# syl051088/DynaAlign

Hardware: AMD Instinct MI355X
Metric: sequence-pairs/sec (MinHash k=4 n_hash=500; NW BLOSUM62) at 1/2/4/8 MI355X (higher is better)
Workload: dtype u32

## Files before the change

### dynaalign_amd/csrc/api.cpp

```cpp
#include <sched.h>

#include <algorithm>
#include <atomic>
#include <chrono>
#include <climits>
#include <cmath>
#include <condition_variable>
#include <cstddef>
#include <map>
#include <memory>
#include <cstdlib>
#include <cstring>
#include <functional>
#include <mutex>
#include <random>
#include <string>
#include <thread>
#include <vector>

#include "da_common.hpp"

namespace da { size_t destroy_cached_comms(); }

namespace da {
// ... 306 lines not shown

double now_ms() { return std::chrono::duration<double, std::milli>(std::chrono::steady_clock::now().time_since_epoch()).count(); }

size_t block_budget() {
  size_t free_b = 0, total_b = 0;
  if (hipMemGetInfo(&free_b, &total_b) != hipSuccess) free_b = (size_t)8 << 30;
  {
    int dev = 0;
    (void)hipGetDevice(&dev);
    std::lock_guard<std::mutex> g(big_cache().m);
    for (const auto &e : big_cache().parked) if (e.dev == dev) free_b += e.bytes;
  }
  size_t budget = free_b / 2;
  if (da::config().block_bytes) budget = (size_t)da::config().block_bytes;
  return budget;
}
int64_t block_rows(int64_t n, size_t bytes_per_elem) {
  int64_t rows = (int64_t)(block_budget() / ((size_t)n * bytes_per_elem));
  rows = rows / 128 * 128;
  if (rows < 128) rows = 128;
  return rows;
}
int64_t rows_per_block(int64_t n, size_t bytes_per_elem) { return std::min(block_rows(n, bytes_per_elem), n); }

}
}

using namespace da;

namespace da {
namespace {
bool env_flag(const char *name) { return getenv(name) != nullptr; }
int64_t env_i64(const char *name, int64_t dflt) { const char *e = getenv(name); return e ? atoll(e) : dflt; }
uint64_t env_u64(const char *name, uint64_t dflt) { const char *e = getenv(name); return e ? strtoull(e, nullptr, 10) : dflt; }
enum MhExpand { MH_EXPAND_DEFAULT, MH_EXPAND_ROWS, MH_EXPAND_ROWSPIPE, MH_EXPAND_PIPE, MH_EXPAND_TILES };
Config parse_config() {
  Config c;
  c.mh_no_dedup = env_flag("DYNAALIGN_MH_NO_DEDUP");
  c.mh_no_sparse = env_flag("DYNAALIGN_MH_NO_SPARSE");
  c.mh_no_pipe = env_flag("DYNAALIGN_MH_NO_PIPE");
  c.mh_pipe_one_stream = env_flag("DYNAALIGN_MH_PIPE_ONE_STREAM");
  c.mh_dedup_min_n = env_i64("DYNAALIGN_MH_DEDUP_MIN_N", -1);
  c.mh_dedup_max_pct = env_i64("DYNAALIGN_MH_DEDUP_MAX_PCT", -1);
  c.mh_sparse_max_pairs = std::min<uint64_t>(env_u64("DYNAALIGN_MH_SPARSE_MAX_PAIRS", 400000000ull), 0xfffffff0ull);
  c.mh_no_hybrid = env_flag("DYNAALIGN_MH_NO_HYBRID");
  c.mh_hybrid_min_n = env_i64("DYNAALIGN_MH_HYBRID_MIN_N", -1);
  c.mh_hybrid_dedup = env_flag("DYNAALIGN_MH_HYBRID_DEDUP");
  if (const char *e = getenv("DYNAALIGN_MH_EXPAND"))
    c.mh_expand = !strcmp(e, "rows") ? MH_EXPAND_ROWS : !strcmp(e, "rowspipe") ? MH_EXPAND_ROWSPIPE : !strcmp(e, "pipe") ? MH_EXPAND_PIPE
                : !strcmp(e, "tiles") ? MH_EXPAND_TILES : MH_EXPAND_DEFAULT;
  c.mh_pipe_step = (int)std::max<int64_t>(0, env_i64("DYNAALIGN_MH_PIPE_STEP", 0));
  c.mh_pipe_wg = (int)std::max<int64_t>(0, std::min<int64_t>(4, env_i64("DYNAALIGN_MH_PIPE_WG", 0)));
  c.mh_pipe_head = (int)std::max<int64_t>(0, env_i64("DYNAALIGN_MH_PIPE_HEAD", 0));
  const int pb = (int)env_i64("DYNAALIGN_PLANE_BITS", 0);
  c.plane_bits = (pb == 32 || pb == 16 || pb == 15 || pb == 14 || pb == 12) ? pb : 0;
  c.k2_no_asm = env_flag("DYNAALIGN_K2_NO_ASM");
  c.k2_persist = env_flag("DYNAALIGN_K2_PERSIST");
  c.k2_wg_per_cu = (int)std::max<int64_t>(0, env_i64("DYNAALIGN_K2_WG_PER_CU", 0));
  c.nw_no_dedup = env_flag("DYNAALIGN_NW_NO_DEDUP");
  c.nw_int32 = env_flag("DYNAALIGN_NW_INT32");
  c.nw_no_prefix = env_flag("DYNAALIGN_NW_NO_PREFIX_SHARE");
  c.nw_dedup_min_n = env_i64("DYNAALIGN_NW_DEDUP_MIN_N", -1);
  c.no_host_widen = env_flag("DYNAALIGN_NO_HOST_WIDEN");
  c.plain_d2h = env_flag("DYNAALIGN_PLAIN_D2H");
  c.no_buffer_cache = env_flag("DYNAALIGN_NO_BUFFER_CACHE");
  c.d2h_threads = (int)std::max<int64_t>(0, env_i64("DYNAALIGN_D2H_THREADS", 0));
  c.buffer_cache_pct = (int)std::max<int64_t>(0, std::min<int64_t>(90, env_i64("DYNAALIGN_BUFFER_CACHE_PCT", 30)));
  c.block_bytes = env_u64("DYNAALIGN_BLOCK_BYTES", 0);
  c.trace = env_flag("DYNAALIGN_TRACE");
  c.louvain_debug = env_flag("DYNAALIGN_LOUVAIN_DEBUG");
  c.louvain_threads = (int)std::max<int64_t>(0, env_i64("DYNAALIGN_LOUVAIN_THREADS", 0));
  return c;
}
std::atomic<const Config *> g_config{nullptr};
}
const Config &config() {
  const Config *c = g_config.load(std::memory_order_acquire);
  if (!c) {
    const Config *fresh = new Config(parse_config());
    if (g_config.compare_exchange_strong(c, fresh, std::memory_order_acq_rel)) c = fresh;
    else delete fresh;
  }
  return *c;
}
}
extern "C" void da_config_reload(void) { da::g_config.store(new da::Config(da::parse_config()), std::memory_order_release); }

extern "C" {

const char *da_last_error(void) { return last_error_ref().c_str(); }

const char *da_status_message(int status) {
  switch (status) {
    case DA_ERR_EMPTY_INPUT: return "Input sequences vector cannot be empty";
    case DA_ERR_BAD_K: return "'k' must be a positive integer";
    case DA_ERR_BAD_NHASH: return "Number of hash functions must be positive";
    case DA_ERR_BAD_MATRIX: return "Invalid substitution matrix name: %s";
    case DA_ERR_BAD_RESIDUE_SEQ1: return "Invalid amino acid in sequence1: %c";
    case DA_ERR_BAD_RESIDUE_SEQ2: return "Invalid amino acid in sequence2: %c";
    case DA_ERR_NOMEM: return "out of memory";
    case DA_ERR_NO_DEVICE: return "no usable HIP device";
    case DA_ERR_HIP: return "HIP runtime error";
    case DA_ERR_UNSUPPORTED: return "unsupported by the gfx950 kernels";
    case DA_ERR_BAD_ARG: return "bad argument";
    default: return "";
  }
// ... 244 lines not shown
  const uint16_t *dense = nullptr, *rare = nullptr;
  unsigned long long st[4] = {0, 0, 0, 0};
  if ((rc = split_ok ? launch_mh_heavy_split(d_work, n, n_hash, dict.max_ids, HY_KEEP, &dense, &rare, d_stats, stream)
                     : launch_mh_sparse_count(ids, ld_ids, n, n_hash, dict.max_ids, d_stats, stream)) != DA_OK) return rc;
  DA_HIP_TRY(hipMemcpyAsync(split_ok ? st : st + 2, d_stats, split_ok ? sizeof(st) : 16, hipMemcpyDeviceToHost, stream));
  DA_HIP_TRY(hipStreamSynchronize(stream));
  const double pairs_all = 0.5 * (double)n * (double)(n - 1);
  if (sparse_ok && st[2] <= mh_sparse_pairs_limit() && st[3] <= 4096 && (double)st[2] <= pairs_all * (double)n_hash / 5000.0)
    *a = MhAdmission{MhOperand::sparse, st[2], ids, nullptr, ld_ids};
  else if (split_ok && st[0] <= mh_sparse_pairs_limit() && st[1] <= 4096 && (double)st[0] <= pairs_all * (double)n_hash / 25000.0)
    *a = MhAdmission{MhOperand::split, st[0], rare, dense, ld_ids};
  return DA_OK;
}
struct MhCodes {
  DevBuf sig, planes, pwork, scratch, entries32, entries;
  int64_t m = 0;
  int n_hash = 0, bits = 32;
  Dictionary dict;
  MhAdmission adm;
  bool split() const { return adm.form == MhOperand::split; }
  int lists(hipStream_t st) const {
    return launch_mh_sparse_lists(adm.codes, adm.ld_ids, m, n_hash, dict.max_ids, adm.pairs, scratch.as<uint32_t>(), entries32.as<uint32_t>(), entries.as<uint16_t>(), st);
  }
  int fixup(int kind, void *out, int64_t ld_out, hipStream_t st, int64_t tr0 = 0, int64_t tr1 = -1) const {
    return launch_mh_sparse_fixup(scratch.as<uint32_t>(), entries.as<uint16_t>(), m, n_hash, dict.max_ids, adm.ld_ids, kind, out, ld_out, tr0,
                                  tr1 < 0 ? (m + 127) / 128 : tr1, st);
  }
};
static int mh_codes(const uint8_t *d_res, const int64_t *d_off, int64_t m, int k, int n_hash, const uint32_t *d_seeds, bool ask_sparse,
                    int split_from_bits, MhCodes *c, hipStream_t stream) {
  int rc;
  const int64_t lds = sig_ld_for(n_hash);
  const size_t wb = mh_planes_workspace_bytes(m, n_hash);
  c->m = m; c->n_hash = n_hash;
  if ((rc = c->sig.alloc((size_t)m * lds * sizeof(uint32_t))) != DA_OK || (rc = c->planes.alloc((size_t)mh_planes_words(m, n_hash) * sizeof(uint32_t))) != DA_OK ||
      (rc = c->pwork.alloc(wb)) != DA_OK) return rc;
  uint32_t *sig = c->sig.as<uint32_t>(), *planes = c->planes.as<uint32_t>();
  if ((rc = launch_minhash_signatures(d_res, d_off, m, k, n_hash, d_seeds, sig, lds, stream)) != DA_OK) return rc;
  const int min_bits = env_plane_bits();
  const Dictionary &dict = c->dict;
  if ((rc = run_dictionary(sig, lds, m, n_hash, min_bits, c->pwork.p, wb, &c->dict, stream)) != DA_OK) return rc;
  if ((rc = mh_admit(dict, c->pwork.p, m, n_hash, ask_sparse, split_from_bits, &c->adm, stream)) != DA_OK) return rc;
  if (c->adm.form != MhOperand::dense &&
      (c->scratch.alloc(mh_sparse_scratch_words(m, n_hash, dict.max_ids, c->adm.ld_ids) * 4) != DA_OK ||
       c->entries32.alloc((size_t)c->adm.pairs * 4 + 16) != DA_OK || c->entries.alloc((size_t)c->adm.pairs * 2 + 16) != DA_OK)) {
    (void)hipGetLastError();
    c->scratch.release(); c->entries32.release(); c->entries.release();
    c->adm = MhAdmission();
  }
  if (c->adm.form == MhOperand::sparse) { c->bits = 0; return DA_OK; }
  if (c->split()) { c->bits = 8; return launch_ids_to_planes(c->pwork.p, m, n_hash, 8, planes, stream, c->adm.dense); }
  return planes_from(dict, sig, lds, m, n_hash, min_bits, c->pwork.p, planes, &c->bits, stream);
}
struct MhCall {
  int64_t n; int n_hash; double *out; int64_t ld; hipStream_t stream; MhRoute &route; const MhEvents &ev; const MhCodes &c; const MhDedup &d;
  uint16_t *dtab = nullptr; int64_t ld_d = 0; void *ex = nullptr; bool pk = false;
};
constexpr int MH_NO_PIPE = -1;
static int mh_finish(const MhCall &k, int last_event, MhForm taken, int steps) {
  DA_HIP_TRY(hipEventRecord(k.ev[last_event], k.stream));
  DA_HIP_TRY(hipStreamSynchronize(k.stream));
  k.route.taken = taken; k.ev.steps(k.route, steps);
  return DA_OK;
}
static int mh_sparse(const MhCall &k) {
  const MhCodes &c = k.c;
  int rc;
  if ((rc = launch_mh_sparse(c.adm.codes, c.adm.ld_ids, k.n, k.n_hash, c.dict.max_ids, c.adm.pairs, c.scratch.as<uint32_t>(), c.entries32.as<uint32_t>(),
                             c.entries.as<uint16_t>(), k.out, k.ld, k.stream, k.ev[3])) != DA_OK || (rc = mh_finish(k, 4, MH_SPARSE, 3)) != DA_OK) return rc;
  k.route.unique = (int64_t)c.adm.pairs;
  MhEvents::ms(k.route, 4, k.ev[3], k.ev[4]);
  return DA_OK;
}
static int mh_direct(const MhCall &k) {
  const MhCodes &c = k.c;
  int rc;
  const PipeLease lease(1, c.split());
  PipeRes *const pr = lease.r;
  if (pr) {
    DA_HIP_TRY(hipStreamWaitEvent(pr->side, k.ev[2], 0));
    if ((rc = c.lists(pr->side)) != DA_OK) return rc;
    DA_HIP_TRY(hipEventRecord(pr->ev[0], pr->side));
  } else if (c.split() && (rc = c.lists(k.stream)) != DA_OK) return rc;
  if ((rc = launch_mh_compare(c.planes.as<uint32_t>(), k.n, k.n_hash, 0, k.n, true, DA_OUT_F64, k.out, k.ld, k.stream, c.bits)) != DA_OK) return rc;
  if (pr) DA_HIP_TRY(hipStreamWaitEvent(k.stream, pr->ev[0], 0));
  if (c.split() && (rc = c.fixup(DA_OUT_F64, k.out, k.ld, k.stream)) != DA_OK) return rc;
  return mh_finish(k, 3, MH_DIRECT, 3);
}
static int mh_one_stream(const MhCall &k) {
  const MhCodes &c = k.c;
  int rc;
  if (c.split() && (rc = c.lists(k.stream)) != DA_OK) return rc;
  if ((rc = k.pk ? launch_mh_compare_pk(c.planes.as<uint32_t>(), k.d.U, k.n_hash, reinterpret_cast<uint8_t *>(k.dtab), k.stream)
                 : launch_mh_compare(c.planes.as<uint32_t>(), k.d.U, k.n_hash, 0, k.d.U, true, DA_OUT_COMPACT, k.dtab, k.ld_d, k.stream, c.bits)) != DA_OK)
    return rc;
  if (c.split() && (rc = c.fixup(DA_OUT_COMPACT, k.dtab, k.ld_d, k.stream)) != DA_OK) return rc;
  DA_HIP_TRY(hipEventRecord(k.ev[3], k.stream));
  if ((rc = k.d.rows ? launch_expand_stream(k.dtab, k.ld_d, k.d.p.uidx, k.n, k.d.U, k.n_hash, k.out, k.ld, k.ex, k.stream, k.ev[4], k.pk)
                     : launch_expand_unique(k.dtab, k.ld_d, k.d.p.uidx, k.n, DA_OUT_F64, false, k.n_hash, k.out, k.ld, k.stream, 0,
                                            static_cast<uint16_t *>(k.ex), k.d.p.ufirst, k.d.U, k.ev[4], k.ev[5])) != DA_OK) return rc;
  k.route.chunks = k.route.expand_launches = 1;
  return k.d.rows ? mh_finish(k, 5, MH_ROWS, 5) : mh_finish(k, 6, MH_TILES, 6);
}
static int mh_rows_pipe(const MhCall &k) {
  const Config &cfg = da::config();
  const MhCodes &c = k.c;
  const int64_t U = k.d.U, KB = mh_sym_bands(U);
  const hipStream_t stream = k.stream;
  int rc;
  const bool two = expand_stream_packed(k.n_hash);
  const int wg = cfg.mh_pipe_wg > 0 ? cfg.mh_pipe_wg : two ? 2 : 1, head = cfg.mh_pipe_head > 0 ? cfg.mh_pipe_head : two ? 1 : 4,
            step = cfg.mh_pipe_step > 0 ? cfg.mh_pipe_step : two ? 8 : 4;
  const bool alt = !cfg.mh_pipe_one_stream;
  std::vector<int64_t> cuts{0};
  while (cuts.back() < KB) cuts.push_back(std::min(KB, cuts.back() + (cuts.size() == 1 ? head : step)));
  const size_t C = cuts.size() - 1;
  const PipeLease lease(3 * C + 2);
  PipeRes *const pr = lease.r;
  if (!pr) return MH_NO_PIPE;
  hipEvent_t *pe = pr->ev.data();
  DA_HIP_TRY(hipStreamWaitEvent(pr->side, k.ev[2], 0));
  if ((rc = launch_mh_compare_edges_u16(c.planes.as<uint32_t>(), U, k.n_hash, k.dtab, k.ld_d, stream, c.bits, k.pk)) != DA_OK) return rc;
  if ((rc = launch_expand_stream_lists(k.d.p.uidx, k.n, U, k.ex, stream)) != DA_OK) return rc;
  DA_HIP_TRY(hipEventRecord(pe[3 * C], stream));
  if (c.split()) {
    if ((rc = c.lists(stream)) != DA_OK) return rc;
    DA_HIP_TRY(hipEventRecord(pe[3 * C + 1], stream));
  }
  if (alt) { DA_HIP_TRY(hipStreamWaitEvent(pr->alt[0], pe[3 * C], 0)); DA_HIP_TRY(hipStreamWaitEvent(pr->alt[1], pe[3 * C], 0)); }
  for (size_t ci = 0; ci < C; ++ci) {
    if ((rc = launch_mh_compare_bands_u16(c.planes.as<uint32_t>(), U, k.n_hash, k.dtab, k.ld_d, cuts[ci], cuts[ci + 1], ci == 0 ? 4 : wg, pr->side, c.bits,
                                          k.pk)) != DA_OK) return rc;
    if (c.split()) {
      if (ci == 0) { DA_HIP_TRY(hipStreamWaitEvent(pr->side, pe[3 * C], 0)); DA_HIP_TRY(hipStreamWaitEvent(pr->side, pe[3 * C + 1], 0)); }
      if ((rc = c.fixup(DA_OUT_COMPACT, k.dtab, k.ld_d, pr->side, cuts[ci] * 8, cuts[ci + 1] * 8)) != DA_OK) return rc;
    }
    DA_HIP_TRY(hipEventRecord(pe[3 * ci], pr->side));
    const hipStream_t es = alt ? pr->alt[ci & 1] : stream;
    DA_HIP_TRY(hipStreamWaitEvent(es, pe[3 * ci], 0));
    DA_HIP_TRY(hipEventRecord(pe[3 * ci + 1], es));
    if ((rc = launch_expand_stream_rows(k.dtab, k.ld_d, k.d.p.uidx, k.n, U, k.n_hash, k.out, k.ld, k.ex, cuts[ci] * 1024, cuts[ci + 1] * 1024, es,
                                        (int)ci, k.pk)) != DA_OK) return rc;
    DA_HIP_TRY(hipEventRecord(pe[3 * ci + 2], es));
  }
  if (alt) for (size_t ci = (C >= 2 ? C - 2 : 0); ci < C; ++ci) DA_HIP_TRY(hipStreamWaitEvent(stream, pe[3 * ci + 2], 0));
  if ((rc = mh_finish(k, 5, MH_ROWS_PIPE, 2)) != DA_OK) return rc;
  k.route.chunks = k.route.expand_launches = (int)C;
  MhEvents::ms(k.route, 2, k.ev[2], pe[3 * (C - 1)]);
  MhEvents::ms(k.route, 3, k.ev[2], pe[3 * C]);
  LaunchUnion expand{k.ev[2]};
  for (size_t ci = 0; ci < C; ++ci) expand.add(pe[3 * ci + 1], pe[3 * ci + 2]);
  k.route.ms[4] = expand.total;
  return DA_OK;
}
static int mh_tiles_pipe(const MhCall &k) {
  const Config &cfg = da::config();
  const MhCodes &c = k.c;
  uint16_t *ftab = static_cast<uint16_t *>(k.ex);
  const hipStream_t stream = k.stream;
  const std::vector<int32_t> &ub = k.d.ub;
  const int64_t U = k.d.U, KB = mh_sym_bands(U), NB = (int64_t)ub.size() - 1, ld_f = ceil_div(k.n, 8) * 8;
  int rc;
  const int step = cfg.mh_pipe_step > 0 ? cfg.mh_pipe_step : 4, wg = cfg.mh_pipe_wg > 0 ? cfg.mh_pipe_wg : 2;
  const bool alt = !cfg.mh_pipe_one_stream;
  struct Chunk { int64_t kb0, kb1, ob0, ob1; };
  std::vector<Chunk> chunks;
  for (int64_t kb = 0, ob = 0; kb < KB;) {
    const int64_t kb1 = std::min(KB, kb + (chunks.empty() ? 1 : step));
    int64_t ob1 = ob;
    if (kb1 == KB) ob1 = NB;
    else while (ob1 < NB && (int64_t)ub[(size_t)ob1 + 1] <= kb1 * 1024) ++ob1;
    chunks.push_back({kb, kb1, ob, ob1});
    kb = kb1; ob = ob1;
  }
  const size_t C = chunks.size();
  const PipeLease lease(5 * C);
  PipeRes *const pr = lease.r;
  if (!pr) return MH_NO_PIPE;
  hipEvent_t *pe = pr->ev.data();
  DA_HIP_TRY(hipStreamWaitEvent(pr->side, k.ev[2], 0));
  if ((rc = launch_mh_compare_edges_u16(c.planes.as<uint32_t>(), U, k.n_hash, k.dtab, k.ld_d, pr->side, c.bits)) != DA_OK) return rc;
  if (c.split() && (rc = c.lists(pr->side)) != DA_OK) return rc;
  for (size_t ci = 0; ci < C; ++ci) {
    const Chunk &ch = chunks[ci];
    if ((rc = launch_mh_compare_bands_u16(c.planes.as<uint32_t>(), U, k.n_hash, k.dtab, k.ld_d, ch.kb0, ch.kb1, wg, pr->side, c.bits)) != DA_OK) return rc;
    if (c.split() && (rc = c.fixup(DA_OUT_COMPACT, k.dtab, k.ld_d, pr->side, ch.kb0 * 8, ch.kb1 * 8)) != DA_OK) return rc;
    DA_HIP_TRY(hipEventRecord(pe[5 * ci], pr->side));
    DA_HIP_TRY(hipStreamWaitEvent(stream, pe[5 * ci], 0));
    DA_HIP_TRY(hipEventRecord(pe[5 * ci + 1], stream));
    if ((rc = launch_gather_columns(k.dtab, k.ld_d, k.d.p.uidx, k.d.p.ufirst, k.n, U, ftab, ld_f, false, stream, 1, 0, ch.kb0 * 1024,
                                    std::min(U, ch.kb1 * 1024))) != DA_OK) return rc;
    DA_HIP_TRY(hipEventRecord(pe[5 * ci + 2], stream));
    const hipStream_t es = alt ? pr->alt[ci & 1] : stream;
    if (alt) DA_HIP_TRY(hipStreamWaitEvent(es, pe[5 * ci + 2], 0));
    DA_HIP_TRY(hipEventRecord(pe[5 * ci + 3], es));
    if ((rc = launch_expand_rows(ftab, ld_f, k.d.p.uidx, k.n, false, k.n_hash, 0, k.out, k.ld, ch.ob0, ch.ob1, es)) != DA_OK) return rc;
    DA_HIP_TRY(hipEventRecord(pe[5 * ci + 4], es));
  }
  if (alt) for (size_t ci = (C >= 2 ? C - 2 : 0); ci < C; ++ci) DA_HIP_TRY(hipStreamWaitEvent(stream, pe[5 * ci + 4], 0));
  DA_HIP_TRY(hipEventRecord(k.ev[5], stream));
  if ((rc = launch_expand_unique(k.dtab, k.ld_d, k.d.p.uidx, k.n, DA_OUT_F64, false, k.n_hash, k.out, k.ld, stream, 0, ftab, k.d.p.ufirst, U,
                                 nullptr, nullptr, 1, 0, true)) != DA_OK) return rc;
  if ((rc = mh_finish(k, 6, MH_TILES_PIPE, 2)) != DA_OK) return rc;
  k.route.chunks = (int)C;
  MhEvents::ms(k.route, 2, k.ev[2], pe[5 * (C - 1)]);
  LaunchUnion expand{k.ev[2]};
  for (size_t ci = 0; ci < C; ++ci) {
    float g = 0;
    (void)hipEventElapsedTime(&g, pe[5 * ci + 1], pe[5 * ci + 2]);
    k.route.ms[3] += g;
    if (chunks[ci].ob1 > chunks[ci].ob0) { ++k.route.expand_launches; expand.add(pe[5 * ci + 3], pe[5 * ci + 4]); }
  }
  k.route.ms[4] = expand.total;
  MhEvents::ms(k.route, 5, k.ev[5], k.ev[6]);
  return DA_OK;
}
}

static int mh_full_symmetric(const uint8_t *d_res, const int64_t *d_off, int64_t n, int64_t total, int k, int n_hash,
                             const uint32_t *d_seeds, double *d_out, int64_t ld, hipStream_t stream) {
  const Config &cfg = da::config();
  int rc;
  MhRoute &route = mh_route() = MhRoute();
  route.n = n;
  MhEvents ev;
  for (auto &e : ev.e) DA_HIP_TRY(hipEventCreate(&e));
  DA_HIP_TRY(hipEventRecord(ev[0], stream));
  MhDedup d;
  if ((rc = mh_dedup_plan(d_res, d_off, n, total, n_hash, d_out, ld, &d, stream)) != DA_OK) return rc;
  route.unique = d.U;
  DA_HIP_TRY(hipEventRecord(ev[1], stream));
  MhCodes c;
  if ((rc = mh_codes(d.take ? d.p.ucodes : d_res, d.take ? d.p.uoff : d_off, d.take ? d.U : n, k, n_hash, d_seeds, !d.take && d.U * 10 >= n * 9,
                     d.take && !cfg.mh_hybrid_dedup ? 13 : 12, &c, stream)) != DA_OK) return rc;
  route.plane_bits = c.bits;
  if (c.split()) { route.hybrid_pairs = (int64_t)c.adm.pairs; route.hybrid_bits_before = c.dict.bits_data; }
  DA_HIP_TRY(hipEventRecord(ev[2], stream));
  MhCall call{n, n_hash, d_out, ld, stream, route, ev, c, d};
  if (!d.take) return c.adm.form == MhOperand::sparse ? mh_sparse(call) : mh_direct(call);
  DevBuf dtab, ex;
  call.pk = d.rows && !c.split() && mh_compare_pk_ok(d.U, n_hash, c.bits);
  route.packed_table = call.pk;
  call.ld_d = call.pk ? pk_lo_bytes(d.U) : (d.U + 7) / 8 * 8;
  if ((rc = dtab.alloc(call.pk ? pk_table_bytes(d.U) : (size_t)d.U * (size_t)call.ld_d * 2)) != DA_OK) return rc;
  if ((rc = ex.alloc(d.rows ? expand_stream_scratch_bytes(n, d.U) : expand_rows_workspace_bytes(n, d.U, DA_OUT_F64, false, n_hash, 0))) != DA_OK) return rc;
  call.dtab = dtab.as<uint16_t>(); call.ex = ex.p;
  const bool pipe = !cfg.mh_no_pipe && mh_compare_bands_ok(d.U, n_hash, c.bits, dtab.p, call.ld_d) &&
                    (d.rows ? cfg.mh_expand != MH_EXPAND_ROWS : cfg.mh_expand != MH_EXPAND_TILES && (ld & 1) == 0 && (reinterpret_cast<uintptr_t>(d_out) & 15) == 0);
  if (pipe && (rc = d.rows ? mh_rows_pipe(call) : mh_tiles_pipe(call)) != MH_NO_PIPE) return rc;
  return mh_one_stream(call);
}

int da_dev_similarity_mh(const uint8_t *d_residues, const int64_t *d_offsets, int64_t n, int64_t total_residues, int k, int n_hash,
                         const uint32_t *d_seeds, double *d_out, int64_t ld, void *stream) {
  int rc = validate_mh(n, k, n_hash);
  if (rc != DA_OK) return rc;
  if (!d_residues || !d_offsets || !d_seeds || !d_out) return fail(DA_ERR_BAD_ARG, "NULL device pointer");
  if (ld < n) return fail(DA_ERR_BAD_ARG, "ld (%lld) < n (%lld)", (long long)ld, (long long)n);
  if (n_hash > 65535) return fail(DA_ERR_UNSUPPORTED, "the compare kernel counts in 16 bits: n_hash <= 65535 (got %d); da_similarity_mh handles more", n_hash);
  return mh_full_symmetric(d_residues, d_offsets, n, total_residues, k, n_hash, d_seeds, d_out, ld, static_cast<hipStream_t>(stream));
}

int da_mh_last_route_chunks(int *chunks_out, int *expand_launches_out) {
  const MhRoute &r = mh_route();
  if (chunks_out) *chunks_out = r.chunks;
  if (expand_launches_out) *expand_launches_out = r.expand_launches;
  return DA_OK;
}

int da_mh_last_route_split(int64_t *rare_incidences_out, int *plane_bits_without_out) {
  const MhRoute &r = mh_route();
  if (rare_incidences_out) *rare_incidences_out = r.hybrid_pairs;
  if (plane_bits_without_out) *plane_bits_without_out = r.hybrid_bits_before;
  return DA_OK;
}

extern "C" int da_debug_mh_last_table_packed(int *packed_out) {
  if (!packed_out) return fail(DA_ERR_BAD_ARG, "NULL pointer");
  *packed_out = mh_route().packed_table ? 1 : 0;
  return DA_OK;
}

int da_mh_last_route(int64_t *n_out, int64_t *unique_out, int *dedup_taken_out, int *plane_bits_out, double *ms6_out) {
  const MhRoute &r = mh_route();
  if (n_out) *n_out = r.n;
  if (unique_out) *unique_out = r.unique;
  if (dedup_taken_out) *dedup_taken_out = r.taken;
  if (plane_bits_out) *plane_bits_out = r.plane_bits;
  if (ms6_out) for (int i = 0; i < 6; ++i) ms6_out[i] = r.ms[i];
  return DA_OK;
}

int da_dev_mh_compare_rect(const uint32_t *d_planes, int plane_bits, int64_t n, int n_hash, int64_t row_begin, int64_t row_end, int64_t col_begin,
                           int64_t col_end, int kind, void *d_out, int64_t ld, void *stream) {
  if (n <= 0) return fail(DA_ERR_EMPTY_INPUT, "%s", da_status_message(DA_ERR_EMPTY_INPUT));
  if (n_hash <= 0) return fail(DA_ERR_BAD_NHASH, "%s", da_status_message(DA_ERR_BAD_NHASH));
  if (!d_planes || !d_out) return fail(DA_ERR_BAD_ARG, "NULL device pointer");
  if (row_begin < 0 || row_end > n || row_begin > row_end) return fail(DA_ERR_BAD_ARG, "bad row range");
  if (col_begin < 0 || col_end > n || col_begin > col_end) return fail(DA_ERR_BAD_ARG, "bad column range");
  if (ld < col_end - col_begin) return fail(DA_ERR_BAD_ARG, "ld (%lld) < columns (%lld)", (long long)ld, (long long)(col_end - col_begin));
  if (kind != DA_OUT_F64 && kind != DA_OUT_COMPACT) return fail(DA_ERR_BAD_ARG, "bad output kind");
  if (n_hash > 65535)
// ... 2344 lines not shown
```

### dynaalign_amd/csrc/da_common.hpp

```cpp
#pragma once

#include <hip/hip_runtime.h>

#include <cstdarg>
#include <cstdint>
#include <cstdio>
#include <string>

#include "../../include/dynaalign.h"

namespace da {
struct Config {
  bool mh_no_dedup = false, mh_no_sparse = false, mh_no_pipe = false, mh_pipe_one_stream = false;
  int64_t mh_dedup_min_n = -1, mh_dedup_max_pct = -1;
  uint64_t mh_sparse_max_pairs = 400000000ull;
  bool mh_no_hybrid = false, mh_hybrid_dedup = false;
  int64_t mh_hybrid_min_n = -1;
  int mh_expand = 0;
  int mh_pipe_step = 0, mh_pipe_wg = 0, mh_pipe_head = 0;
  int plane_bits = 0;
  bool k2_no_asm = false, k2_persist = false;
  int k2_wg_per_cu = 0;
  bool nw_no_dedup = false, nw_int32 = false, nw_no_prefix = false;
  int64_t nw_dedup_min_n = -1;
  bool no_host_widen = false, plain_d2h = false, no_buffer_cache = false;
  int d2h_threads = 0, buffer_cache_pct = 30;
  uint64_t block_bytes = 0;
  bool trace = false, louvain_debug = false;
  int louvain_threads = 0;
};
const Config &config();


std::string &last_error_ref();
int fail(int code, const char *fmt, ...) __attribute__((format(printf, 2, 3)));

#define DA_HIP_TRY(expr)                                                              \
  do {                                                                                \
    hipError_t _e = (expr);                                                           \
    if (_e != hipSuccess)                                                             \
      return ::da::fail(_e == hipErrorNoDevice || _e == hipErrorInvalidDevice         \
                            ? DA_ERR_NO_DEVICE                                        \
                            : DA_ERR_HIP,                                             \
                        "%s failed: %s (%s:%d)", #expr, hipGetErrorString(_e),        \
                        __FILE__, __LINE__);                                          \
  } while (0)

inline int64_t ceil_div(int64_t a, int64_t b) { return (a + b - 1) / b; }

struct ShardGeom {
  int64_t n, W, rows;
  int world, tile, T, Q, Qh;
};
__host__ __device__ inline int64_t shard_back(int64_t W, int64_t n) { return W - ((n + 7) / 8) * 8; }
inline ShardGeom shard_geom(int64_t n, int world, int tile) {
  ShardGeom g;
  g.n = n; g.world = world; g.tile = tile;
  g.T = (int)ceil_div(n, tile);
  g.Q = (int)ceil_div(g.T, world);
  g.Qh = (g.Q + 1) / 2;
  g.W = ceil_div(n, 8) * 8 + (int64_t)world * tile;
  g.rows = (int64_t)g.Qh * tile;
  return g;
}

__host__ __device__ inline int k2_slot(int r) { return (((r >> 5) * 2 + (r & 1)) << 4) + ((r & 31) >> 1); }
__host__ __device__ inline int k2_row_of_slot(int s) { return ((s >> 5) << 5) + ((s & 15) << 1) + ((s >> 4) & 1); }
struct PlaneGeom {
  int pl;
  int sp;
  int segs;
  int nst;
// ... 20 lines not shown
__host__ __device__ inline int64_t pad16_slot_word(int64_t n, int n_hash, int64_t row, int group) {
  const int64_t nst = (n_hash + 31) / 32;
  return (((row >> 7) * nst + group) * 128 + k2_slot((int)(row & 127))) * K2_PAD16_SLOT_WORDS;
}
inline int64_t mh_planes_words(int64_t n, int n_hash) {
  if (n <= 0 || n_hash <= 0) return 0;
  const int64_t raw = 2 * plane_geom(n, n_hash, 32).copy_words;
  const int64_t p16 = pad16_base_words(n, n_hash) + 2 * pad16_copy_words(n, n_hash);
  return raw > p16 ? raw : p16;
}

__host__ __device__ inline int64_t pk_lo_bytes(int64_t U) { return (U + 127) / 128 * 128; }
__host__ __device__ inline int64_t pk_row_bytes(int64_t lo_bytes) { return lo_bytes + lo_bytes / 8; }
inline size_t pk_table_bytes(int64_t U) { return (size_t)U * (size_t)pk_row_bytes(pk_lo_bytes(U)); }

constexpr int TK_PER = 8;

__device__ __forceinline__ uint32_t wave_incl_scan(uint32_t v) {
  const int lane = threadIdx.x & 63;
#pragma unroll
  for (int o = 1; o < 64; o <<= 1) {
    const uint32_t t = __shfl_up(v, o);
    if (lane >= o) v += t;
  }
  return v;
}

__device__ __forceinline__ int load8(const uint16_t *__restrict__ row, int64_t j0, int64_t n, bool vec, const uint16_t *__restrict__ rank,
                                     uint32_t r[TK_PER], uint32_t k[TK_PER]) {
  int nv;
  if (vec && j0 + TK_PER <= n) {
    const uint4 v = *reinterpret_cast<const uint4 *>(row + j0);
    const uint32_t w[4] = {v.x, v.y, v.z, v.w};
#pragma unroll
    for (int e = 0; e < TK_PER; ++e) k[e] = (w[e >> 1] >> ((e & 1) * 16)) & 0xFFFFu;
    nv = TK_PER;
  } else {
    nv = j0 >= n ? 0 : (n - j0 < TK_PER ? (int)(n - j0) : TK_PER);
#pragma unroll
    for (int e = 0; e < TK_PER; ++e) k[e] = e < nv ? (uint32_t)row[j0 + e] : 0u;
  }
#pragma unroll
  for (int e = 0; e < TK_PER; ++e) r[e] = (rank && e < nv) ? (uint32_t)rank[k[e]] : k[e];
  return nv;
}

int launch_minhash_signatures(const uint8_t *d_res, const int64_t *d_off, int64_t n,
                              int k, int n_hash, const uint32_t *d_seeds, uint32_t *d_sig,
                              int64_t ld_sig, hipStream_t stream);
int launch_mh_compare(const uint32_t *d_planes, int64_t n, int n_hash,
                      int64_t row_begin, int64_t row_end, bool symmetric, int kind,
                      void *d_out, int64_t ld, hipStream_t stream, int plane_bits = 32, int tile_stride = 1,
                      bool upper_only = false, int fold_q = 0, int64_t fold_w = 0);
int launch_mh_compare_rect(const uint32_t *d_planes, int64_t n, int n_hash, int64_t row_begin, int64_t row_end, int64_t col_begin, int64_t col_end,
                           int kind, void *d_out, int64_t ld, hipStream_t stream, int plane_bits);
int launch_fill_sig_rows(uint32_t *d_sig, int64_t ld_sig, int64_t m, int64_t m_pad, int n_hash, hipStream_t stream);
int64_t mh_sym_bands(int64_t n);
int64_t mh_sym_band_prefix(int64_t n, int64_t band);
bool mh_compare_bands_ok(int64_t n, int n_hash, int plane_bits, const void *d_out, int64_t ld);
int launch_mh_compare_bands_u16(const uint32_t *d_planes, int64_t n, int n_hash, uint16_t *d_out, int64_t ld, int64_t band_begin,
                                int64_t band_end, int wg_per_cu, hipStream_t stream, int plane_bits = 12, bool pk = false);
int launch_mh_compare_edges_u16(const uint32_t *d_planes, int64_t n, int n_hash, uint16_t *d_out, int64_t ld, hipStream_t stream, int plane_bits = 12,
                                bool pk = false);
bool mh_compare_pk_ok(int64_t n, int n_hash, int plane_bits);
int launch_mh_compare_pk(const uint32_t *d_planes, int64_t n, int n_hash, uint8_t *d_tab, hipStream_t stream);
size_t mh_sparse_pairs_limit();
int launch_mh_sparse_count(const uint16_t *d_idsT, int64_t ld_ids, int64_t n, int n_hash, int max_ids, unsigned long long *d_stats, hipStream_t stream);
size_t mh_sparse_scratch_words(int64_t n, int n_hash, int max_ids, int64_t ld_ids);
int launch_mh_sparse(const uint16_t *d_idsT, int64_t ld_ids, int64_t n, int n_hash, int max_ids, uint64_t pairs, uint32_t *d_scratch,
                     uint32_t *d_entries32, uint16_t *d_entries, double *d_out, int64_t ld, hipStream_t stream, hipEvent_t after_buckets = nullptr);
int launch_mh_sparse_lists(const uint16_t *d_idsT, int64_t ld_ids, int64_t n, int n_hash, int max_ids, uint64_t pairs, uint32_t *d_scratch,
                           uint32_t *d_entries32, uint16_t *d_entries, hipStream_t stream);
int launch_mh_sparse_fixup(const uint32_t *d_scratch, const uint16_t *d_entries, int64_t n, int n_hash, int max_ids, int64_t ld_ids, int kind, void *d_out,
                           int64_t ld, int64_t tile_row_begin, int64_t tile_row_end, hipStream_t stream);
const uint16_t *mh_dictionary_codes(const void *d_work, int64_t n, int n_hash, int64_t *ld_ids);
constexpr int64_t DA_DICT_MAX_N = 131068;
size_t mh_planes_workspace_bytes(int64_t n, int n_hash);
int launch_mh_dictionary(const uint32_t *d_sig, int64_t ld_sig, int64_t n, int n_hash, void *d_work,
                         int **d_status_out, hipStream_t stream);
int mh_plane_bits_for(int max_ids);
int launch_ids_to_planes(const void *d_work, int64_t n, int n_hash, int plane_bits, uint32_t *d_planes,
                         hipStream_t stream, const uint16_t *d_codes = nullptr);
int launch_mh_heavy_split(void *d_work, int64_t n, int n_hash, int max_ids, int keep, const uint16_t **d_dense_out, const uint16_t **d_sparse_out,
                          unsigned long long *d_stats, hipStream_t stream);
int launch_sig_to_planes(const uint32_t *d_sig, int64_t ld_sig, int64_t n, int n_hash, uint32_t *d_planes,
                         hipStream_t stream);
int launch_finalize_sharded(const uint16_t *d_g, int64_t ld_g, const ShardGeom &geom, bool is_nw, int n_hash,
                            double *d_out, int64_t ld, hipStream_t stream);
int64_t shard_packed_bytes(const ShardGeom &g, int value_bits);
int launch_shards_to_table(const void *d_g, int64_t ld_g, const ShardGeom &geom, int value_bits, uint16_t *d_table, int64_t ld,
                           hipStream_t stream);
int launch_pack_shard(const uint16_t *d_local, int64_t ld, const ShardGeom &geom, int value_bits, uint8_t *d_packed,
                      hipStream_t stream);
int launch_finalize_packed(const uint8_t *d_g, const ShardGeom &geom, int value_bits, int n_hash, double *d_out, int64_t ld,
                           hipStream_t stream);
int launch_nw_encode(const uint8_t *d_res, int64_t total, uint8_t *d_codes, int32_t *d_bad,
                     hipStream_t stream);
int launch_nw(const uint8_t *d_codes, const int64_t *d_off, int64_t n, int64_t max_len,
              int matrix_id, int gap_open, int gap_ext, int64_t row_begin, int64_t row_end,
              bool symmetric, int kind, void *d_out, int64_t ld, int32_t *d_score,
              int64_t ld_score, hipStream_t stream, int shard_rank = 0, int shard_world = 0,
              const int32_t *ord_first = nullptr, const int32_t *ord_minfirst = nullptr, const int32_t *ord_maxlast = nullptr,
              const int32_t *ord_perm = nullptr, const uint8_t *ord_lcp = nullptr,
              int64_t col_begin = 0, int64_t col_end = -1);
size_t nw_sort_unique_workspace_bytes(int64_t n);
int launch_nw_sort_unique(const uint8_t *d_codes, const int64_t *d_off, int64_t n, void *d_work, size_t work_bytes, const int32_t **perm_out,
// ... 87 lines not shown
```

### dynaalign_amd/csrc/minhash_kernels.hip

```cpp
#include "da_common.hpp"

#include <algorithm>
#include <atomic>
#include <mutex>
#include <vector>
#include <type_traits>

namespace da {
namespace {

__device__ __forceinline__ uint32_t rotl32(uint32_t v, int r) {
  return __builtin_rotateleft32(v, r);
}
__device__ __forceinline__ uint32_t mm3_scramble(uint32_t w) {
  w *= 0xcc9e2d51u;
  w = rotl32(w, 15);
  w *= 0x1b873593u;
  return w;
}
__device__ __forceinline__ uint32_t mm3_mix(uint32_t h, uint32_t kk) {
  h ^= kk;
  return rotl32(h, 13) * 5u + 0xe6546b64u;
}
__device__ __forceinline__ uint32_t mm3_final(uint32_t h, uint32_t len) {
// ... 1054 lines not shown
  for (int64_t i = (int64_t)blockIdx.x * blockDim.x + threadIdx.x; i < count; i += stride)
    acc[i] = (first ? 0u : acc[i]) + cnt[i];
}
__global__ __launch_bounds__(256) void k_counts32_to_f64(const uint32_t *__restrict__ acc, double *__restrict__ out, int64_t count, int n_hash) {
  const int64_t stride = (int64_t)gridDim.x * blockDim.x;
  for (int64_t i = (int64_t)blockIdx.x * blockDim.x + threadIdx.x; i < count; i += stride)
    out[i] = (double)acc[i] / (double)n_hash;
}

}

int launch_acc_counts(uint32_t *d_acc, const uint16_t *d_cnt, int64_t count, bool first, hipStream_t stream) {
  if (count <= 0) return DA_OK;
  hipLaunchKernelGGL(k_acc_counts, dim3(256 * 16), dim3(256), 0, stream, d_acc, d_cnt, count, first ? 1 : 0);
  DA_HIP_TRY(hipGetLastError());
  return DA_OK;
}
int launch_counts32_to_f64(const uint32_t *d_acc, double *d_out, int64_t count, int n_hash, hipStream_t stream) {
  if (count <= 0) return DA_OK;
  hipLaunchKernelGGL(k_counts32_to_f64, dim3(256 * 16), dim3(256), 0, stream, d_acc, d_out, count, n_hash);
  DA_HIP_TRY(hipGetLastError());
  return DA_OK;
}

#ifdef DA_K2_TIMING
extern "C" int da_debug_set_k2_timing(unsigned long long *d_buf) {
  return (int)hipMemcpyToSymbol(HIP_SYMBOL(g_k2_timing), &d_buf, sizeof(d_buf));
}
#endif

int launch_minhash_signatures(const uint8_t *d_res, const int64_t *d_off, int64_t n, int k,
                              int n_hash, const uint32_t *d_seeds, uint32_t *d_sig,
                              int64_t ld_sig, hipStream_t stream) {
  if (n <= 0) return DA_OK;
  if (n > 0x7fffffffLL) return fail(DA_ERR_UNSUPPORTED, "more than 2^31-1 sequences");
  const size_t lds = 2 * (size_t)(K1_CHUNK + k) * sizeof(uint32_t);
  if (lds > 64 * 1024) return fail(DA_ERR_UNSUPPORTED, "k = %d is larger than the signature kernel supports (k <= 7168)", k);
  dim3 grid((unsigned)n), block(K1_THREADS);
  if (k == 4)
    hipLaunchKernelGGL(k_minhash_signatures<true>, grid, block, lds, stream, d_res, d_off, k, n_hash, d_seeds, d_sig, ld_sig);
  else
    hipLaunchKernelGGL(k_minhash_signatures<false>, grid, block, lds, stream, d_res, d_off, k, n_hash, d_seeds, d_sig, ld_sig);
  DA_HIP_TRY(hipGetLastError());
  return DA_OK;
}

template <auto V, auto... MORE, typename X, typename F>
static void dispatch(X x, F &&f) {
  if constexpr (sizeof...(MORE) == 0) f(std::integral_constant<decltype(V), V>{});
  else if (x == V) f(std::integral_constant<decltype(V), V>{});
  else dispatch<MORE...>(x, f);
}

int launch_mh_compare(const uint32_t *d_planes, int64_t n, int n_hash,
                      int64_t row_begin, int64_t row_end, bool symmetric, int kind,
                      void *d_out, int64_t ld, hipStream_t stream, int plane_bits, int tile_stride, bool upper_only,
                      int fold_q, int64_t fold_w) {
  if (row_end <= row_begin) return DA_OK;
  if (plane_bits != 8 && plane_bits != 12 && plane_bits != 14 && plane_bits != 15 && plane_bits != 16 && plane_bits != 32)
    return fail(DA_ERR_BAD_ARG, "plane_bits must be 8, 12, 14, 15, 16 or 32 (got %d)", plane_bits);
  const int code_bits = plane_bits;
  if (plane_bits == 14 || plane_bits == 15) plane_bits = 16;
  const int T = (int)ceil_div(n, K2_TILE);
  const int TR = (int)ceil_div(ceil_div(row_end - row_begin, K2_TILE), tile_stride);
  const int64_t ntiles = count_tiles(TR, T, symmetric);
  const int64_t per_xcd = ceil_div(ntiles, 8);
  int band = K2_BAND;
  while (band > 1 && ceil_div(TR, band) < 48) band >>= 1;
  const int64_t nblocks = symmetric ? per_xcd * 8 : 8 * ceil_div(ceil_div(TR, band), 8) * (int64_t)band * T;
  if (nblocks > 0x7fffffffLL) return fail(DA_ERR_UNSUPPORTED, "pair space too large for one launch");
  dim3 grid((unsigned)nblocks), block(K2_THREADS);
  const bool f64 = kind == DA_OUT_F64, asm_ok = !config().k2_no_asm && k2_out_ok(d_out, ld, f64);
  const bool a12 = symmetric && plane_bits == 12 && asm_ok && (!f64 || (int64_t)n_hash + 1 <= K2_A12_TABLE_MAX);
  const bool a16 = symmetric && plane_bits == 16 && asm_ok && (!f64 || (int64_t)n_hash + 1 <= K2_A16_TABLE_MAX);
  const bool a8 = symmetric && plane_bits == 8 && asm_ok && n_hash > K2_GROUP && (!f64 || n_hash < K2_P8_TABLE) && per_xcd < 0x7fffffffLL;
  const bool s12 = !symmetric && plane_bits == 12 && kind == DA_OUT_COMPACT && asm_ok && (row_begin % K2_TILE) == 0;
  const bool s16 = !symmetric && plane_bits == 16 && kind == DA_OUT_COMPACT && asm_ok && (row_begin % K2_TILE) == 0;
  if (a8)
    dispatch<false, true>(f64, [&](auto F64) {
      if (config().k2_persist) {
        int wg_per_xcd = 4 * 32;
        if (config().k2_wg_per_cu > 0) wg_per_xcd = config().k2_wg_per_cu * 32;
        if ((int64_t)wg_per_xcd > per_xcd) wg_per_xcd = (int)(per_xcd > 0 ? per_xcd : 1);
        hipLaunchKernelGGL((k_mh_compare_p12<decltype(F64)::value, 8, false>), dim3((unsigned)(8 * wg_per_xcd)), block, 0, stream, d_planes, n, n_hash,
                           d_out, ld, ntiles, per_xcd, wg_per_xcd, (int64_t)0);
      } else {
        hipLaunchKernelGGL((k_mh_compare_p12<decltype(F64)::value, 8, true>), grid, block, 0, stream, d_planes, n, n_hash, d_out, ld, ntiles, per_xcd,
                           (int)per_xcd, (int64_t)0);
      }
    });
  if (a16)
    dispatch<false, true>(f64, [&](auto F64) {
      dispatch<14, 15, 16>(code_bits, [&](auto B) {
        hipLaunchKernelGGL((k_mh_compare_a16<decltype(F64)::value, decltype(B)::value>), grid, block, 0, stream, d_planes, n, n_hash, d_out, ld, ntiles,
                           per_xcd);
      });
    });
  const bool p12 = a12 && n_hash > K2_GROUP && (!f64 || n_hash < K2_P12_TABLE) && config().k2_persist;
  if (p12) {
    static std::atomic<int> occ_cache[2], cus_cache;
    const int ki = kind == DA_OUT_F64 ? 0 : 1;
    if (!occ_cache[ki].load()) {
      int occ = 0;
      if (ki == 0) DA_HIP_TRY(hipOccupancyMaxActiveBlocksPerMultiprocessor(&occ, k_mh_compare_p12<true>, K2_THREADS, 0));
      else DA_HIP_TRY(hipOccupancyMaxActiveBlocksPerMultiprocessor(&occ, k_mh_compare_p12<false>, K2_THREADS, 0));
      int dev = 0;
      hipDeviceProp_t prop;
      DA_HIP_TRY(hipGetDevice(&dev));
      DA_HIP_TRY(hipGetDeviceProperties(&prop, dev));
      if (config().k2_wg_per_cu > 0) occ = config().k2_wg_per_cu;
      cus_cache.store(prop.multiProcessorCount > 0 ? prop.multiProcessorCount : 256);
      occ_cache[ki].store(occ > 0 ? occ : 1);
      if (config().trace)
        fprintf(stderr, "[dynaalign] k_mh_compare_p12<%s>: %d resident workgroups per CU, %d CUs\n", ki == 0 ? "f64" : "u16", occ_cache[ki].load(), cus_cache.load());
    }
    int wg_per_xcd = occ_cache[ki].load() * ((cus_cache.load() + 7) / 8);
    if ((int64_t)wg_per_xcd > per_xcd) wg_per_xcd = (int)(per_xcd > 0 ? per_xcd : 1);
    const dim3 pgrid((unsigned)(8 * wg_per_xcd));
    if (kind == DA_OUT_F64)
      hipLaunchKernelGGL(k_mh_compare_p12<true>, pgrid, block, 0, stream, d_planes, n, n_hash, d_out, ld, ntiles, per_xcd, wg_per_xcd, (int64_t)0);
    else
      hipLaunchKernelGGL(k_mh_compare_p12<false>, pgrid, block, 0, stream, d_planes, n, n_hash, d_out, ld, ntiles, per_xcd, wg_per_xcd, (int64_t)0);
  } else if (a12) {
    if (f64)
      hipLaunchKernelGGL(k_mh_compare_a12<true>, grid, block, 0, stream, d_planes, n, n_hash, d_out, ld, ntiles, per_xcd);
    else
      hipLaunchKernelGGL(k_mh_compare_a12<false>, grid, block, 0, stream, d_planes, n, n_hash, d_out, ld, ntiles, per_xcd);
  }
  if (s12)
// ... 1357 lines not shown
```

Measured before the change: 334.9 billion.

## Add front-rows table and early expand lists to overlap rows pipeline head

```diff
diff --git a/dynaalign_amd/csrc/api.cpp b/dynaalign_amd/csrc/api.cpp
--- a/dynaalign_amd/csrc/api.cpp
+++ b/dynaalign_amd/csrc/api.cpp
@@ -382,6 +382,8 @@
   c.mh_pipe_step = (int)std::max<int64_t>(0, env_i64("DYNAALIGN_MH_PIPE_STEP", 0));
   c.mh_pipe_wg = (int)std::max<int64_t>(0, std::min<int64_t>(4, env_i64("DYNAALIGN_MH_PIPE_WG", 0)));
   c.mh_pipe_head = (int)std::max<int64_t>(0, env_i64("DYNAALIGN_MH_PIPE_HEAD", 0));
+  c.mh_pipe_front = (int)std::max<int64_t>(-1, std::min<int64_t>(4096, env_i64("DYNAALIGN_MH_PIPE_FRONT", -1)));
+  c.mh_pipe_wg0 = (int)std::max<int64_t>(0, std::min<int64_t>(4, env_i64("DYNAALIGN_MH_PIPE_WG0", 0)));
   const int pb = (int)env_i64("DYNAALIGN_PLANE_BITS", 0);
   c.plane_bits = (pb == 32 || pb == 16 || pb == 15 || pb == 14 || pb == 12) ? pb : 0;
   c.k2_no_asm = env_flag("DYNAALIGN_K2_NO_ASM");
@@ -732,9 +734,27 @@
   if (c->split()) { c->bits = 8; return launch_ids_to_planes(c->pwork.p, m, n_hash, 8, planes, stream, c->adm.dense); }
   return planes_from(dict, sig, lds, m, n_hash, min_bits, c->pwork.p, planes, &c->bits, stream);
 }
+struct RowsPipeHead {
+  enum { LISTS_DONE, SPLIT_LISTS, LISTS_BEGIN, EDGES, FRONT_TABLE, FRONT_BEGIN, FRONT_END, NAMED };
+  std::vector<int64_t> cuts{0};
+  PipeRes *pr = nullptr;
+  bool lists_early = false;
+  size_t chunks() const { return cuts.size() - 1; }
+  size_t events() const { return 3 * chunks() + NAMED; }
+  hipEvent_t ev(int named) const { return pr->ev[3 * chunks() + (size_t)named]; }
+  void plan(int64_t U, int n_hash) {
+    const Config &cfg = da::config();
+    const bool two = expand_stream_packed(n_hash);
+    const int64_t KB = mh_sym_bands(U), head = cfg.mh_pipe_head > 0 ? cfg.mh_pipe_head : two ? 1 : 4,
+                  step = cfg.mh_pipe_step > 0 ? cfg.mh_pipe_step : two ? 8 : 4;
+    while (cuts.back() < KB) cuts.push_back(std::min(KB, cuts.back() + (cuts.size() == 1 ? head : step)));
+  }
+};
 struct MhCall {
   int64_t n; int n_hash; double *out; int64_t ld; hipStream_t stream; MhRoute &route; const MhEvents &ev; const MhCodes &c; const MhDedup &d;
   uint16_t *dtab = nullptr; int64_t ld_d = 0; void *ex = nullptr; bool pk = false;
+  const RowsPipeHead *head = nullptr;
+  DevBuf *front = nullptr;
 };
 constexpr int MH_NO_PIPE = -1;
 static int mh_finish(const MhCall &k, int last_event, MhForm taken, int steps) {
@@ -783,52 +803,75 @@
   return k.d.rows ? mh_finish(k, 5, MH_ROWS, 5) : mh_finish(k, 6, MH_TILES, 6);
 }
 static int mh_rows_pipe(const MhCall &k) {
+  using H = RowsPipeHead;
   const Config &cfg = da::config();
   const MhCodes &c = k.c;
-  const int64_t U = k.d.U, KB = mh_sym_bands(U);
+  const H &h = *k.head;
+  const int64_t U = k.d.U;
   const hipStream_t stream = k.stream;
   int rc;
-  const bool two = expand_stream_packed(k.n_hash);
-  const int wg = cfg.mh_pipe_wg > 0 ? cfg.mh_pipe_wg : two ? 2 : 1, head = cfg.mh_pipe_head > 0 ? cfg.mh_pipe_head : two ? 1 : 4,
-            step = cfg.mh_pipe_step > 0 ? cfg.mh_pipe_step : two ? 8 : 4;
+  PipeRes *const pr = h.pr;
+  if (!pr) return MH_NO_PIPE;
+  const std::vector<int64_t> &cuts = h.cuts;
+  const size_t C = h.chunks();
+  hipEvent_t *pe = pr->ev.data();
+  const int wg = cfg.mh_pipe_wg > 0 ? cfg.mh_pipe_wg : expand_stream_packed(k.n_hash) ? 2 : 1, wg0 = cfg.mh_pipe_wg0 > 0 ? cfg.mh_pipe_wg0 : 4;
   const bool alt = !cfg.mh_pipe_one_stream;
-  std::vector<int64_t> cuts{0};
-  while (cuts.back() < KB) cuts.push_back(std::min(KB, cuts.back() + (cuts.size() == 1 ? head : step)));
-  const size_t C = cuts.size() - 1;
-  const PipeLease lease(3 * C + 2);
-  PipeRes *const pr = lease.r;
-  if (!pr) return MH_NO_PIPE;
-  hipEvent_t *pe = pr->ev.data();
+  const int64_t R = std::min(U, cfg.mh_pipe_front < 0 ? 256 : ceil_div((int64_t)cfg.mh_pipe_front, 128) * 128), ld_f = ceil_div(U, 8) * 8;
+  bool front = R > 0 && !c.split() && c.bits == 12;
+  if (front && k.front->alloc((size_t)R * (size_t)ld_f * 2) != DA_OK) { (void)hipGetLastError(); front = false; }
+  front = front && mh_compare_rows_s12_ok(c.bits, 0, k.front->p, ld_f);
   DA_HIP_TRY(hipStreamWaitEvent(pr->side, k.ev[2], 0));
+  if (front) {
+    if ((rc = launch_mh_compare(c.planes.as<uint32_t>(), U, k.n_hash, 0, R, false, DA_OUT_COMPACT, k.front->p, ld_f, stream, 12)) != DA_OK) return rc;
+    DA_HIP_TRY(hipEventRecord(h.ev(H::FRONT_TABLE), stream));
+  }
   if ((rc = launch_mh_compare_edges_u16(c.planes.as<uint32_t>(), U, k.n_hash, k.dtab, k.ld_d, stream, c.bits, k.pk)) != DA_OK) return rc;
-  if ((rc = launch_expand_stream_lists(k.d.p.uidx, k.n, U, k.ex, stream)) != DA_OK) return rc;
-  DA_HIP_TRY(hipEventRecord(pe[3 * C], stream));
+  DA_HIP_TRY(hipEventRecord(h.ev(H::EDGES), stream));
+  if (!h.lists_early) {
+    DA_HIP_TRY(hipEventRecord(h.ev(H::LISTS_BEGIN), stream));
+    if ((rc = launch_expand_stream_lists(k.d.p.uidx, k.n, U, k.ex, stream)) != DA_OK) return rc;
+    DA_HIP_TRY(hipEventRecord(h.ev(H::LISTS_DONE), stream));
+  } else if (!alt) DA_HIP_TRY(hipStreamWaitEvent(stream, h.ev(H::LISTS_DONE), 0));
   if (c.split()) {
     if ((rc = c.lists(stream)) != DA_OK) return rc;
-    DA_HIP_TRY(hipEventRecord(pe[3 * C + 1], stream));
-  }
-  if (alt) { DA_HIP_TRY(hipStreamWaitEvent(pr->alt[0], pe[3 * C], 0)); DA_HIP_TRY(hipStreamWaitEvent(pr->alt[1], pe[3 * C], 0)); }
+    DA_HIP_TRY(hipEventRecord(h.ev(H::SPLIT_LISTS), stream));
+  }
+  if (alt) { DA_HIP_TRY(hipStreamWaitEvent(pr->alt[0], h.ev(H::LISTS_DONE), 0)); DA_HIP_TRY(hipStreamWaitEvent(pr->alt[1], h.ev(H::LISTS_DONE), 0)); }
+  if (front) {
+    const hipStream_t fs = alt ? pr->alt[1] : stream;
+    if (alt) DA_HIP_TRY(hipStreamWaitEvent(fs, h.ev(H::FRONT_TABLE), 0));
+    DA_HIP_TRY(hipEventRecord(h.ev(H::FRONT_BEGIN), fs));
+    if ((rc = launch_expand_stream_rows(k.front->as<uint16_t>(), ld_f, k.d.p.uidx, k.n, U, k.n_hash, k.out, k.ld, k.ex, 0, R, fs, (int)C, false)) != DA_OK)
+      return rc;
+    DA_HIP_TRY(hipEventRecord(h.ev(H::FRONT_END), fs));
+  }
+  if (alt && h.lists_early) { DA_HIP_TRY(hipStreamWaitEvent(pr->alt[0], h.ev(H::EDGES), 0)); DA_HIP_TRY(hipStreamWaitEvent(pr->alt[1], h.ev(H::EDGES), 0)); }
+  const int64_t r0 = front ? R : 0;
   for (size_t ci = 0; ci < C; ++ci) {
-    if ((rc = launch_mh_compare_bands_u16(c.planes.as<uint32_t>(), U, k.n_hash, k.dtab, k.ld_d, cuts[ci], cuts[ci + 1], ci == 0 ? 4 : wg, pr->side, c.bits,
+    if ((rc = launch_mh_compare_bands_u16(c.planes.as<uint32_t>(), U, k.n_hash, k.dtab, k.ld_d, cuts[ci], cuts[ci + 1], ci == 0 ? wg0 : wg, pr->side, c.bits,
                                           k.pk)) != DA_OK) return rc;
     if (c.split()) {
-      if (ci == 0) { DA_HIP_TRY(hipStreamWaitEvent(pr->side, pe[3 * C], 0)); DA_HIP_TRY(hipStreamWaitEvent(pr->side, pe[3 * C + 1], 0)); }
+      if (ci == 0) { DA_HIP_TRY(hipStreamWaitEvent(pr->side, h.ev(H::EDGES), 0)); DA_HIP_TRY(hipStreamWaitEvent(pr->side, h.ev(H::SPLIT_LISTS), 0)); }
       if ((rc = c.fixup(DA_OUT_COMPACT, k.dtab, k.ld_d, pr->side, cuts[ci] * 8, cuts[ci + 1] * 8)) != DA_OK) return rc;
     }
     DA_HIP_TRY(hipEventRecord(pe[3 * ci], pr->side));
     const hipStream_t es = alt ? pr->alt[ci & 1] : stream;
     DA_HIP_TRY(hipStreamWaitEvent(es, pe[3 * ci], 0));
     DA_HIP_TRY(hipEventRecord(pe[3 * ci + 1], es));
-    if ((rc = launch_expand_stream_rows(k.dtab, k.ld_d, k.d.p.uidx, k.n, U, k.n_hash, k.out, k.ld, k.ex, cuts[ci] * 1024, cuts[ci + 1] * 1024, es,
-                                        (int)ci, k.pk)) != DA_OK) return rc;
+    if ((rc = launch_expand_stream_rows(k.dtab, k.ld_d, k.d.p.uidx, k.n, U, k.n_hash, k.out, k.ld, k.ex, std::max(r0, cuts[ci] * 1024), cuts[ci + 1] * 1024,
+                                        es, (int)ci, k.pk)) != DA_OK) return rc;
     DA_HIP_TRY(hipEventRecord(pe[3 * ci + 2], es));
   }
   if (alt) for (size_t ci = (C >= 2 ? C - 2 : 0); ci < C; ++ci) DA_HIP_TRY(hipStreamWaitEvent(stream, pe[3 * ci + 2], 0));
+  if (alt && front) DA_HIP_TRY(hipStreamWaitEvent(stream, h.ev(H::FRONT_END), 0));
   if ((rc = mh_finish(k, 5, MH_ROWS_PIPE, 2)) != DA_OK) return rc;
-  k.route.chunks = k.route.expand_launches = (int)C;
+  k.route.chunks = (int)C;
+  k.route.expand_launches = (int)C + (front ? 1 : 0);
   MhEvents::ms(k.route, 2, k.ev[2], pe[3 * (C - 1)]);
-  MhEvents::ms(k.route, 3, k.ev[2], pe[3 * C]);
+  MhEvents::ms(k.route, 3, h.ev(H::LISTS_BEGIN), h.ev(H::LISTS_DONE));
   LaunchUnion expand{k.ev[2]};
+  if (front) expand.add(h.ev(H::FRONT_BEGIN), h.ev(H::FRONT_END));
   for (size_t ci = 0; ci < C; ++ci) expand.add(pe[3 * ci + 1], pe[3 * ci + 2]);
   k.route.ms[4] = expand.total;
   return DA_OK;
@@ -911,6 +954,21 @@
   route.unique = d.U;
   DA_HIP_TRY(hipEventRecord(ev[1], stream));
   MhCodes c;
+  DevBuf dtab, ex, front;
+  RowsPipeHead head;
+  const bool rows_pipe = d.take && d.rows && !cfg.mh_no_pipe && cfg.mh_expand != MH_EXPAND_ROWS;
+  if (rows_pipe) head.plan(d.U, n_hash);
+  const PipeLease lease(head.events(), rows_pipe);
+  head.pr = lease.r;
+  if (d.take && (rc = ex.alloc(d.rows ? expand_stream_scratch_bytes(n, d.U) : expand_rows_workspace_bytes(n, d.U, DA_OUT_F64, false, n_hash, 0))) != DA_OK)
+    return rc;
+  if (head.pr && cfg.mh_pipe_front != 0) {
+    DA_HIP_TRY(hipStreamWaitEvent(head.pr->side, ev[1], 0));
+    DA_HIP_TRY(hipEventRecord(head.ev(RowsPipeHead::LISTS_BEGIN), head.pr->side));
+    if ((rc = launch_expand_stream_lists(d.p.uidx, n, d.U, ex.p, head.pr->side)) != DA_OK) return rc;
+    DA_HIP_TRY(hipEventRecord(head.ev(RowsPipeHead::LISTS_DONE), head.pr->side));
+    head.lists_early = true;
+  }
   if ((rc = mh_codes(d.take ? d.p.ucodes : d_res, d.take ? d.p.uoff : d_off, d.take ? d.U : n, k, n_hash, d_seeds, !d.take && d.U * 10 >= n * 9,
                      d.take && !cfg.mh_hybrid_dedup ? 13 : 12, &c, stream)) != DA_OK) return rc;
   route.plane_bits = c.bits;
@@ -918,16 +976,15 @@
   DA_HIP_TRY(hipEventRecord(ev[2], stream));
   MhCall call{n, n_hash, d_out, ld, stream, route, ev, c, d};
   if (!d.take) return c.adm.form == MhOperand::sparse ? mh_sparse(call) : mh_direct(call);
-  DevBuf dtab, ex;
   call.pk = d.rows && !c.split() && mh_compare_pk_ok(d.U, n_hash, c.bits);
   route.packed_table = call.pk;
   call.ld_d = call.pk ? pk_lo_bytes(d.U) : (d.U + 7) / 8 * 8;
   if ((rc = dtab.alloc(call.pk ? pk_table_bytes(d.U) : (size_t)d.U * (size_t)call.ld_d * 2)) != DA_OK) return rc;
-  if ((rc = ex.alloc(d.rows ? expand_stream_scratch_bytes(n, d.U) : expand_rows_workspace_bytes(n, d.U, DA_OUT_F64, false, n_hash, 0))) != DA_OK) return rc;
-  call.dtab = dtab.as<uint16_t>(); call.ex = ex.p;
+  call.dtab = dtab.as<uint16_t>(); call.ex = ex.p; call.head = &head; call.front = &front;
   const bool pipe = !cfg.mh_no_pipe && mh_compare_bands_ok(d.U, n_hash, c.bits, dtab.p, call.ld_d) &&
                     (d.rows ? cfg.mh_expand != MH_EXPAND_ROWS : cfg.mh_expand != MH_EXPAND_TILES && (ld & 1) == 0 && (reinterpret_cast<uintptr_t>(d_out) & 15) == 0);
   if (pipe && (rc = d.rows ? mh_rows_pipe(call) : mh_tiles_pipe(call)) != MH_NO_PIPE) return rc;
+  if (head.lists_early) DA_HIP_TRY(hipStreamWaitEvent(stream, head.ev(RowsPipeHead::LISTS_DONE), 0));
   return mh_one_stream(call);
 }
 
diff --git a/dynaalign_amd/csrc/da_common.hpp b/dynaalign_amd/csrc/da_common.hpp
--- a/dynaalign_amd/csrc/da_common.hpp
+++ b/dynaalign_amd/csrc/da_common.hpp
@@ -18,6 +18,7 @@
   int64_t mh_hybrid_min_n = -1;
   int mh_expand = 0;
   int mh_pipe_step = 0, mh_pipe_wg = 0, mh_pipe_head = 0;
+  int mh_pipe_front = -1, mh_pipe_wg0 = 0;
   int plane_bits = 0;
   bool k2_no_asm = false, k2_persist = false;
   int k2_wg_per_cu = 0;
@@ -144,6 +145,7 @@
                       int64_t row_begin, int64_t row_end, bool symmetric, int kind,
                       void *d_out, int64_t ld, hipStream_t stream, int plane_bits = 32, int tile_stride = 1,
                       bool upper_only = false, int fold_q = 0, int64_t fold_w = 0);
+bool mh_compare_rows_s12_ok(int plane_bits, int64_t row_begin, const void *d_out, int64_t ld);
 int launch_mh_compare_rect(const uint32_t *d_planes, int64_t n, int n_hash, int64_t row_begin, int64_t row_end, int64_t col_begin, int64_t col_end,
                            int kind, void *d_out, int64_t ld, hipStream_t stream, int plane_bits);
 int launch_fill_sig_rows(uint32_t *d_sig, int64_t ld_sig, int64_t m, int64_t m_pad, int n_hash, hipStream_t stream);
diff --git a/dynaalign_amd/csrc/minhash_kernels.hip b/dynaalign_amd/csrc/minhash_kernels.hip
--- a/dynaalign_amd/csrc/minhash_kernels.hip
+++ b/dynaalign_amd/csrc/minhash_kernels.hip
@@ -1130,6 +1130,9 @@
   else dispatch<MORE...>(x, f);
 }
 
+bool mh_compare_rows_s12_ok(int plane_bits, int64_t row_begin, const void *d_out, int64_t ld) {
+  return plane_bits == 12 && !config().k2_no_asm && k2_out_ok(d_out, ld, false) && (row_begin % K2_TILE) == 0;
+}
 int launch_mh_compare(const uint32_t *d_planes, int64_t n, int n_hash,
                       int64_t row_begin, int64_t row_end, bool symmetric, int kind,
                       void *d_out, int64_t ld, hipStream_t stream, int plane_bits, int tile_stride, bool upper_only,
@@ -1152,7 +1155,7 @@
   const bool a12 = symmetric && plane_bits == 12 && asm_ok && (!f64 || (int64_t)n_hash + 1 <= K2_A12_TABLE_MAX);
   const bool a16 = symmetric && plane_bits == 16 && asm_ok && (!f64 || (int64_t)n_hash + 1 <= K2_A16_TABLE_MAX);
   const bool a8 = symmetric && plane_bits == 8 && asm_ok && n_hash > K2_GROUP && (!f64 || n_hash < K2_P8_TABLE) && per_xcd < 0x7fffffffLL;
-  const bool s12 = !symmetric && plane_bits == 12 && kind == DA_OUT_COMPACT && asm_ok && (row_begin % K2_TILE) == 0;
+  const bool s12 = !symmetric && kind == DA_OUT_COMPACT && mh_compare_rows_s12_ok(plane_bits, row_begin, d_out, ld);
   const bool s16 = !symmetric && plane_bits == 16 && kind == DA_OUT_COMPACT && asm_ok && (row_begin % K2_TILE) == 0;
   if (a8)
     dispatch<false, true>(f64, [&](auto F64) {
```

Result: slower. 303.8 billion (-9.3%).
